# craftsangjae/instance-segmentation-road-project

Hardware: AMD Instinct MI355X
Metric: images/sec at 1024x1024 (MaskLab inference hot path, full forward) (higher is better)
Workload: dtype f32; 1 GPU; resnext50_full_b8_1024; per_gpu_batch=8, global_batch=8, height=1024, width=1024, parallelism=dp1, hipgraph=False, inputs=resident in HBM, weights=random init (cls logits x8 so NMS / mask head run at full load)

## Files before the change

include/masklab_hip.h:

```cpp
#ifndef MASKLAB_HIP_H
#define MASKLAB_HIP_H

#include <stdint.h>

#ifdef __cplusplus
extern "C" {
#endif

#define ML_OK 0
#define ML_E_BADARG (-1)
#define ML_E_LAUNCH (-2)
#define ML_E_NOGPU  (-3)

enum { ML_ACT_NONE = 0, ML_ACT_RELU = 1, ML_ACT_RELU6 = 2, ML_ACT_SIGMOID = 3 };
enum { ML_MATH_F32 = 0, ML_MATH_F16 = 1, ML_MATH_F16S = 2, ML_MATH_F32X3 = 3 };

#define ML_ABI_VERSION 7
int ml_version(void);
const char *ml_last_error(void);
int ml_device_check(void);

typedef struct ml_conv2d_desc {
    const float *in;
    const float *wgt;
// ... 93 lines not shown
                              int32_t B, int32_t H, int32_t W, int32_t C, int32_t in_cstride, int32_t in_coff,
                              int32_t Ho, int32_t Wo, int32_t add_cstride, int32_t add_coff,
                              int32_t out_cstride, int32_t out_coff, void *stream);
int ml_dwconv3x3_f16(const void *in, const float *wgt, const float *bias, void *out,
                     int32_t B, int32_t H, int32_t W, int32_t C, int32_t in_cstride, int32_t in_coff,
                     int32_t out_cstride, int32_t out_coff, int32_t Ho, int32_t Wo,
                     int32_t stride, int32_t dil, int32_t pad_t, int32_t pad_l, int32_t act, void *stream);
int ml_global_mean_f16(const void *in, void *out, int32_t B, int32_t HW, int32_t C, void *stream);

int ml_stem7x7s2_pool_f16(const float *image, const void *wgt_h, const float *bias, void *out, int32_t B, int32_t H,
                          int32_t W, int32_t Hp, int32_t Wp, void *stream);
int ml_stem7x7s2_pool_f32(const float *image, const float *wgt, const float *bias, float *out, int32_t B, int32_t H,
                          int32_t W, int32_t Hp, int32_t Wp, void *stream);
int ml_stem7x7s2_pool_x3(const float *image, const void *wgt_x3, const float *bias, float *out, int32_t B, int32_t H,
                         int32_t W, int32_t Hp, int32_t Wp, void *stream);

typedef struct ml_deconv_out_problem {
    const float *x, *wd, *bd, *wo_table, *bo;
    float *out;
    int64_t M;
    int32_t hw, w, rois_per_image, reserved0;
    int64_t out_image_stride, out_base;
    const int32_t *live;
} ml_deconv_out_problem;
int ml_deconv2x2_out1x1_f32(const ml_deconv_out_problem *probs, int32_t nprob, int32_t K, int32_t c_mid, int32_t ncls,
                            int32_t cp, int32_t act_mid, int32_t act_out, void *stream);
int ml_deconv2x2_out1x1_f16(const ml_deconv_out_problem *probs, int32_t nprob, int32_t K, int32_t c_mid, int32_t ncls,
                            int32_t cp, int32_t act_mid, int32_t act_out, void *stream);
int ml_deconv2x2_out1x1_tape_f32(const ml_deconv_out_problem *probs, float *const *tapes, int32_t nprob, int32_t K,
                                 int32_t c_mid, int32_t ncls, int32_t cp, int32_t act_mid, int32_t act_out, void *stream);
// ... 407 lines not shown
```

instance-segmentation-road-project_amd/csrc/common.h:

```cpp
#pragma once
#include <hip/hip_runtime.h>
#include <stdint.h>
#include <stdio.h>
#include "masklab_hip.h"

typedef float f32x2 __attribute__((ext_vector_type(2)));
typedef float f32x4 __attribute__((ext_vector_type(4)));
typedef float f32x16 __attribute__((ext_vector_type(16)));

typedef _Float16 f16x2 __attribute__((ext_vector_type(2)));
typedef _Float16 f16x4 __attribute__((ext_vector_type(4)));
typedef _Float16 f16x8 __attribute__((ext_vector_type(8)));

typedef unsigned u32x2 __attribute__((ext_vector_type(2)));
typedef unsigned u32x4 __attribute__((ext_vector_type(4)));
typedef int i32x4 __attribute__((ext_vector_type(4)));

void ml_set_error(const char *fmt, ...);

#define ML_REQUIRE(cond, ...)                 \
    do {                                      \
        if (!(cond)) {                        \
            ml_set_error(__VA_ARGS__);        \
            return ML_E_BADARG;               \
// ... 31 lines not shown
            : "+v"(lw[i]) : "v"(hw[i]), "s"(neg_scale), "v"(sv[2 * i + 1]));
    }
    const u32x4 H = {hw[0], hw[1], hw[2], hw[3]}, L = {lw[0], lw[1], lw[2], lw[3]};
    hi = __builtin_bit_cast(f16x8, H);
    lo = __builtin_bit_cast(f16x8, L);
}

__device__ __forceinline__ void split_hi_lo_pair(const float xa, const float xb, const float neg_scale, unsigned &hi, unsigned &lo) {
    const f32x2 x = {xa, xb};
    const f32x2 sc = x * 2048.f;
    hi = __builtin_bit_cast(unsigned, __builtin_convertvector(x, f16x2));
    asm("v_fma_mixlo_f16 %0, %1, %2, %3 op_sel_hi:[1,0,0]" : "=v"(lo) : "v"(hi), "s"(neg_scale), "v"(sc[0]));
    asm("v_fma_mixhi_f16 %0, %1, %2, %3 op_sel:[1,0,0] op_sel_hi:[1,0,0]" : "+v"(lo) : "v"(hi), "s"(neg_scale), "v"(sc[1]));
}

static inline bool ml_aligned16(const void *p) { return (((uintptr_t)p) & 15u) == 0; }

#include <atomic>
static inline int ml_ensure_dynamic_lds(const void *fn, int bytes, std::atomic<unsigned long long> &done,
                                        const char *what) {
    int dev = 0;
    hipError_t e = hipGetDevice(&dev);
    if (e != hipSuccess || dev < 0 || dev >= 64) {
        ml_set_error("%s: hipGetDevice failed or device index %d out of range", what, dev);
        return ML_E_LAUNCH;
    }
    const unsigned long long bit = 1ull << dev;
    if (done.load(std::memory_order_acquire) & bit) return ML_OK;
    e = hipFuncSetAttribute(fn, hipFuncAttributeMaxDynamicSharedMemorySize, bytes);
    if (e != hipSuccess) {
// ... 21 lines not shown
```

instance-segmentation-road-project_amd/csrc/pointwise.hip:

```cpp
#include "common.h"

namespace {

constexpr int TPB = 256;

inline unsigned grid_for(long long n) { return (unsigned)((n + TPB - 1) / TPB); }

struct Affine3 { float m[3], d[3], s[3]; };

__global__ void preprocess_kernel(const void *in, int is_u8, float *out, long long npix, int out_c,
                                  int flip, Affine3 a) {
    const long long i = (long long)blockIdx.x * TPB + threadIdx.x;
    if (i >= npix) return;
    float v[3];
    if (is_u8) {
        const unsigned char *p = reinterpret_cast<const unsigned char *>(in) + i * 3;
        v[0] = p[0]; v[1] = p[1]; v[2] = p[2];
    } else {
        const float *p = reinterpret_cast<const float *>(in) + i * 3;
        v[0] = p[0]; v[1] = p[1]; v[2] = p[2];
    }
    if (flip) { const float t = v[0]; v[0] = v[2]; v[2] = t; }
    const float r0 = (v[0] - a.m[0]) / a.d[0] + a.s[0];
    const float r1 = (v[1] - a.m[1]) / a.d[1] + a.s[1];
    const float r2 = (v[2] - a.m[2]) / a.d[2] + a.s[2];
    if (out_c == 4) {
        f32x4 o = {r0, r1, r2, 0.f};
        *reinterpret_cast<f32x4 *>(out + i * 4) = o;
    } else {
        out[i * 3 + 0] = r0; out[i * 3 + 1] = r1; out[i * 3 + 2] = r2;
    }
}

template <class T> constexpr int VEC = 16 / (int)sizeof(T);

template <class T, int N>
__device__ __forceinline__ void load_f(const T *p, float (&v)[N]) {
    typedef T Tv __attribute__((ext_vector_type(VEC<T>)));
#pragma unroll
    for (int k = 0; k < N / VEC<T>; ++k) {
// ... 378 lines not shown
```

instance-segmentation-road-project_amd/csrc/stem.hip:

```cpp
#include <type_traits>
#include "common.h"

namespace {

constexpr int PTH = 4, PTW = 16;
constexpr int NT = 256;
constexpr int CR = 2 * PTH + 1, CC = 2 * PTW + 1;
constexpr int IR = 2 * (CR - 1) + 7;
constexpr int ICP = 2 * (CC - 1) + 8;
constexpr int NCONV = CR * CC;
constexpr int NSETS = (NCONV + 31) / 32;
constexpr int NIN = (IR * ICP + NT - 1) / NT;
static_assert(NSETS == 10, "the wave -> set map below assumes 10 sets");


struct StemF32 {
    typedef float Wgt;
    typedef float Conv;
    static constexpr bool PAIRED = true;
    static constexpr int CPS = 68;
    static constexpr int IN_BYTES = IR * ICP * 3 * 4;
    float wv[7][4][3];
    __device__ __forceinline__ StemF32(const float *wgt, int nt, int p32, int q) {
#pragma unroll
// ... 124 lines not shown
#pragma unroll
        for (int u = 0; u < NS; ++u) {
            const _Float16 *src = reinterpret_cast<const _Float16 *>(lds) + (ip[u] + 2 * q) * 4;
#pragma unroll
            for (int ky = 0; ky < 7; ++ky) {
                f16x8 xv[2];
#pragma unroll
                for (int s2 = 0; s2 < 2; ++s2) xv[s2] = *reinterpret_cast<const f16x8 *>(src + (ky * ICP + 4 * s2) * 4);
#pragma unroll
                for (int s2 = 0; s2 < 2; ++s2) acc[u] = __builtin_amdgcn_mfma_f32_32x32x16_f16(wv[ky * 2 + s2], xv[s2], acc[u], 0, 0, 0);
            }
        }
    }
};

template <class Math>
constexpr int STEM_LDS = Math::IN_BYTES + NSETS * 32 * Math::CPS * (int)sizeof(typename Math::Conv);

template <class Math>
__device__ __forceinline__ void stem_pool_body(const float *img, const typename Math::Wgt *wgt, const float *bias,
                                               typename Math::Conv *out, int H, int W, int Hc, int Wc, int Hp, int Wp,
                                               int tiles_x, int seg) {
    typedef typename Math::Conv CT;
    typedef CT CTx4 __attribute__((ext_vector_type(4)));
    constexpr int V = 16 / sizeof(CT), NG = 64 / V;
    typedef CT CTxV __attribute__((ext_vector_type(V)));
    constexpr int CPS = Math::CPS;
    extern __shared__ __align__(16) char lds[];
    CT *tconv = reinterpret_cast<CT *>(lds + Math::IN_BYTES);

    const int tid = threadIdx.x, lane = tid & 63, wave = tid >> 6;
    const int p32 = lane & 31, q = lane >> 5;
    const int ty = blockIdx.x, b = blockIdx.y;
    const int py0 = ty * PTH;
    const int cy0 = 2 * py0 - 1;
    const int iy0 = 2 * cy0 - 3;
    const int nt = wave >> 1, s0 = wave & 1;

    const Math m(wgt, nt, p32, q);
    float bv[16];
#pragma unroll
    for (int e = 0; e < 16; ++e) bv[e] = bias ? bias[nt * 32 + (e & 3) + 8 * (e >> 2) + 4 * q] : 0.f;

    int in_c[NIN];
    long long in_off[NIN];
#pragma unroll
    for (int j = 0; j < NIN; ++j) {
        const int i = tid + NT * j;
        const int in_r = i / ICP;
        in_c[j] = i - in_r * ICP;
        const int iy = iy0 + in_r;
        const bool row_ok = i < IR * ICP && (unsigned)iy < (unsigned)H;
        in_off[j] = row_ok ? ((long long)(b * H + iy) * W) * 4 : -1;
    }
    f32x4 stage[NIN];
    auto fetch = [&](int tx) __attribute__((always_inline)) {
        const int ix0 = 2 * (2 * tx * PTW - 1) - 3;
#pragma unroll
        for (int j = 0; j < NIN; ++j) {
            const int ix = ix0 + in_c[j];
            f32x4 v = {0.f, 0.f, 0.f, 0.f};
            if (in_off[j] >= 0 && (unsigned)ix < (unsigned)W) v = *reinterpret_cast<const f32x4 *>(img + in_off[j] + (long long)ix * 4);
            stage[j] = v;
        }
    };
    auto conv_sets = [&](auto nc, int sa, int cx0) __attribute__((always_inline)) {
        constexpr int NS = decltype(nc)::value;
        int ip[NS];
        f32x16 acc[NS];
#pragma unroll
        for (int u = 0; u < NS; ++u) {
            const int cp = min((sa + 2 * u) * 32 + p32, NCONV - 1);
            const int cyl = cp / CC, cxl = cp - cyl * CC;
            ip[u] = (2 * cyl) * ICP + 2 * cxl;
#pragma unroll
            for (int e = 0; e < 16; ++e) acc[u][e] = bv[e];
        }
        m.template products<NS>(lds, ip, q, acc);
// ... 5 lines not shown
            const int cy = cy0 + cyl, cx = cx0 + cxl;
            const bool inside = (unsigned)cy < (unsigned)Hc && (unsigned)cx < (unsigned)Wc;
            CT *dst = tconv + (s * 32 + p32) * CPS + nt * 32 + 4 * q;
#pragma unroll
            for (int e4 = 0; e4 < 4; ++e4) {
                CTx4 v;
#pragma unroll
                for (int e = 0; e < 4; ++e) v[e] = inside ? (CT)fmaxf(acc[u][4 * e4 + e], 0.f) : (CT)0.f;
                *reinterpret_cast<CTx4 *>(dst + 8 * e4) = v;
            }
        }
    };

    const int tx_begin = blockIdx.z * seg, tx_end = min(tiles_x, tx_begin + seg);
    fetch(tx_begin);
    m.deposit(lds, stage, tid);
    __syncthreads();
    for (int tx = tx_begin; tx < tx_end; ++tx) {
        const int px0 = tx * PTW;
        const int cx0 = 2 * px0 - 1;
        if (tx + 1 < tx_end) fetch(tx + 1);

        if constexpr (Math::PAIRED) {
            conv_sets(std::integral_constant<int, 2>{}, s0, cx0);
            conv_sets(std::integral_constant<int, 2>{}, s0 + 4, cx0);
            conv_sets(std::integral_constant<int, 1>{}, s0 + 8, cx0);
        } else {
            for (int s = s0; s < NSETS; s += 2) conv_sets(std::integral_constant<int, 1>{}, s, cx0);
        }
        __syncthreads();

        for (int i = tid; i < PTH * PTW * NG; i += NT) {
            const int cg = i & (NG - 1), pp = i / NG;
            const int ppy = pp / PTW, ppx = pp - ppy * PTW;
            const int oy = py0 + ppy, ox = px0 + ppx;
            if (oy >= Hp || ox >= Wp) continue;
            CTxV mx = *reinterpret_cast<const CTxV *>(tconv + ((2 * ppy) * CC + 2 * ppx) * CPS + cg * V);
#pragma unroll
            for (int dy = 0; dy < 3; ++dy)
#pragma unroll
                for (int dx = 0; dx < 3; ++dx) {
                    if (dy == 0 && dx == 0) continue;
                    const CTxV v = *reinterpret_cast<const CTxV *>(tconv + ((2 * ppy + dy) * CC + 2 * ppx + dx) * CPS + cg * V);
#pragma unroll
                    for (int k = 0; k < V; ++k) mx[k] = v[k] > mx[k] ? v[k] : mx[k];
                }
            *reinterpret_cast<CTxV *>(out + ((long long)(b * Hp + oy) * Wp + ox) * 64 + cg * V) = mx;
        }
        if (tx + 1 < tx_end) m.deposit(lds, stage, tid);
        __syncthreads();
    }
}

__global__ void __launch_bounds__(NT, 1)
stem_pool_f32_kernel(const float *__restrict__ img, const float *__restrict__ wgt, const float *__restrict__ bias,
                     float *__restrict__ out, int H, int W, int Hc, int Wc, int Hp, int Wp, int tiles_x, int seg) {
    stem_pool_body<StemF32>(img, wgt, bias, out, H, W, Hc, Wc, Hp, Wp, tiles_x, seg);
}

__global__ void __launch_bounds__(NT, 1)
stem_pool_x3_kernel(const float *__restrict__ img, const _Float16 *__restrict__ wgt, const float *__restrict__ bias,
                    float *__restrict__ out, int H, int W, int Hc, int Wc, int Hp, int Wp, int tiles_x, int seg) {
    stem_pool_body<StemX3>(img, wgt, bias, out, H, W, Hc, Wc, Hp, Wp, tiles_x, seg);
}

__global__ void __launch_bounds__(NT)
stem_pool_h_kernel(const float *__restrict__ img, const _Float16 *__restrict__ wgt, const float *__restrict__ bias,
                   _Float16 *__restrict__ out, int H, int W, int Hc, int Wc, int Hp, int Wp, int tiles_x, int seg) {
    stem_pool_body<StemH>(img, wgt, bias, out, H, W, Hc, Wc, Hp, Wp, tiles_x, seg);
}

template <class Math>
int stem_pool_launch(void (*kernel)(const float *, const typename Math::Wgt *, const float *, typename Math::Conv *, int, int,
                                    int, int, int, int, int, int),
                     const char *name, const float *image, const void *wgt, const float *bias, void *out, int B, int H, int W,
                     int Hp, int Wp, void *stream) {
    constexpr bool wgt_scalar = std::is_same<typename Math::Wgt, float>::value;
    ML_REQUIRE(image && wgt && out, "%s: null pointer", name);
    ML_REQUIRE(B > 0 && B < 65536 && H > 0 && W > 0, "%s: bad dims", name);
    ML_REQUIRE(ml_aligned16(image) && (wgt_scalar || ml_aligned16(wgt)) && ml_aligned16(out), "%s: %s must be 16-byte aligned",
               name, wgt_scalar ? "image and output" : "pointers");
    const int Hc = (H + 6 - 7) / 2 + 1, Wc = (W + 6 - 7) / 2 + 1;
    ML_REQUIRE(Hp == (Hc + 2 - 3) / 2 + 1 && Wp == (Wc + 2 - 3) / 2 + 1,
               "%s: output must be [B, %d, %d, 64] (ZeroPadding2D(1) + MaxPooling2D(3, 2))", name, (Hc + 2 - 3) / 2 + 1,
               (Wc + 2 - 3) / 2 + 1);
    ML_REQUIRE((long long)B * H * W < (1ll << 31), "%s: too many pixels", name);
    static std::atomic<unsigned long long> lds_ok{0};
    if (int rc = ml_ensure_dynamic_lds(reinterpret_cast<const void *>(kernel), STEM_LDS<Math>, lds_ok, name)) return rc;
    const int tiles_y = (Hp + PTH - 1) / PTH, tiles_x = (Wp + PTW - 1) / PTW;
    int seg = tiles_x;
    while (seg > 1 && (long long)tiles_y * B * ((tiles_x + seg - 1) / seg) < 2ll * ml_resident_blocks(1)) seg = (seg + 1) / 2;
    hipLaunchKernelGGL(kernel, dim3(tiles_y, B, (tiles_x + seg - 1) / seg), dim3(NT), STEM_LDS<Math>, (hipStream_t)stream, image,
                       reinterpret_cast<const typename Math::Wgt *>(wgt), bias, reinterpret_cast<typename Math::Conv *>(out), H, W,
                       Hc, Wc, Hp, Wp, tiles_x, seg);
    ML_CHECK_LAUNCH(name);
    return ML_OK;
}

}

extern "C" int ml_stem7x7s2_pool_f32(const float *image, const float *wgt, const float *bias, float *out, int32_t B, int32_t H,
                                     int32_t W, int32_t Hp, int32_t Wp, void *stream) {
    return stem_pool_launch<StemF32>(stem_pool_f32_kernel, "stem7x7s2_pool_f32", image, wgt, bias, out, B, H, W, Hp, Wp, stream);
}

extern "C" int ml_stem7x7s2_pool_x3(const float *image, const void *wgt_x3, const float *bias, float *out, int32_t B, int32_t H,
                                    int32_t W, int32_t Hp, int32_t Wp, void *stream) {
    return stem_pool_launch<StemX3>(stem_pool_x3_kernel, "stem7x7s2_pool_x3", image, wgt_x3, bias, out, B, H, W, Hp, Wp, stream);
}

extern "C" int ml_stem7x7s2_pool_f16(const float *image, const void *wgt_h, const float *bias, void *out, int32_t B, int32_t H,
                                     int32_t W, int32_t Hp, int32_t Wp, void *stream) {
    return stem_pool_launch<StemH>(stem_pool_h_kernel, "stem7x7s2_pool", image, wgt_h, bias, out, B, H, W, Hp, Wp, stream);
}
```

instance-segmentation-road-project_amd/masklab_hip/_lib.py:

```python
import ctypes as C
import os

_HERE = os.path.dirname(os.path.abspath(__file__))
LIB_PATH = os.path.join(_HERE, "libmasklab_hip.so")

ABI_VERSION = 7
ACT_NONE, ACT_RELU, ACT_RELU6, ACT_SIGMOID = 0, 1, 2, 3
ACT_BY_NAME = {None: ACT_NONE, "linear": ACT_NONE, "relu": ACT_RELU, "relu6": ACT_RELU6,
               "sigmoid": ACT_SIGMOID}


class ConvDesc(C.Structure):
    _fields_ = [
        ("in_", C.c_void_p), ("wgt", C.c_void_p), ("bias", C.c_void_p),
        ("residual", C.c_void_p), ("out", C.c_void_p),
        ("B", C.c_int32), ("H", C.c_int32), ("W", C.c_int32),
        ("in_cstride", C.c_int32), ("in_coff", C.c_int32),
        ("span", C.c_int32), ("span_pad", C.c_int32), ("cpp_shift", C.c_int32),
        ("Ho", C.c_int32), ("Wo", C.c_int32),
        ("KH", C.c_int32), ("KW", C.c_int32), ("stride", C.c_int32), ("dil", C.c_int32),
        ("pad_t", C.c_int32), ("pad_l", C.c_int32),
        ("cout", C.c_int32), ("n_pad", C.c_int32),
        ("out_cstride", C.c_int32), ("out_coff", C.c_int32),
        ("res_cstride", C.c_int32), ("res_coff", C.c_int32),
# ... 130 lines not shown
    "ml_dwconv3x3_dgrad_multi_f32": (C.c_int, [C.POINTER(DwGradDesc), _i32, _vp]),
    "ml_relu_grad_f32": (C.c_int, [_vp, _vp, _vp, _i64, _vp]),
    "ml_deconv2x2_out1x1_f32": (C.c_int, [C.POINTER(DeconvOutProblem), _i32, _i32, _i32, _i32, _i32, _i32, _i32, _vp]),
    "ml_deconv2x2_out1x1_tape_f32": (C.c_int, [C.POINTER(DeconvOutProblem), C.POINTER(C.c_void_p)] + [_i32] * 7 + [_vp]),
    "ml_deconv2x2_out1x1_grad_f32": (C.c_int, [C.POINTER(DeconvOutGradProblem), _i32, _i32, _vp, _i64, _vp]),
    "ml_deconv2x2_out1x1_grad_plan": (C.c_int, [C.POINTER(DeconvOutGradProblem), _i32, C.POINTER(C.c_int32), C.POINTER(C.c_int32),
                                                C.POINTER(C.c_int64)]),
    "ml_deconv2x2_grad_relayout_f32": (C.c_int, [_vp, _vp, _vp, _vp, _i32, _i32, _vp]),
    "ml_gconv3x3_f32": (C.c_int, [_vp, _vp, _vp, _vp] + [_i32] * 11 + [_vp]),
    "ml_gconv3x3_f16": (C.c_int, [_vp, _vp, _vp, _vp] + [_i32] * 11 + [_vp]),
    "ml_gconv3x3_launch_plan": (C.c_int, [_i32] * 9 + [C.POINTER(C.c_int32)]),
    "ml_maxpool3x3s2_f16": (C.c_int, [_vp, _vp] + [_i32] * 8 + [_vp]),
    "ml_stem7x7s2_pool_f16": (C.c_int, [_vp, _vp, _vp, _vp] + [_i32] * 5 + [_vp]),
    "ml_stem7x7s2_pool_f32": (C.c_int, [_vp, _vp, _vp, _vp] + [_i32] * 5 + [_vp]),
    "ml_stem7x7s2_pool_x3": (C.c_int, [_vp, _vp, _vp, _vp] + [_i32] * 5 + [_vp]),
    "ml_subsample2_f16": (C.c_int, [_vp, _vp] + [_i32] * 4 + [_vp]),
    "ml_cast_f16_to_f32": (C.c_int, [_vp, _vp, _i64, _vp]),
    "ml_cast_f32_to_f16": (C.c_int, [_vp, _vp, _i64, _vp]),
    "ml_resize_bilinear_ac_f16": (C.c_int, [_vp, _vp, _vp] + [_i32] * 12 + [_vp]),
    "ml_dwconv3x3_f16": (C.c_int, [_vp, _vp, _vp, _vp] + [_i32] * 15 + [_vp]),
    "ml_global_mean_f16": (C.c_int, [_vp, _vp, _i32, _i32, _i32, _vp]),
    "ml_groupnorm_chunk_f16": (C.c_int, [_vp, _vp, _vp, _vp, _i32, _i64, _i32, _i32, _f32, _i32, _i32, _i32, _vp, _vp]),
    "ml_roi_crop_resize_f16": (C.c_int, [_vp, _vp, _i32, _i32, _vp, _vp, _vp, _vp] + [_i32] * 10 + [_f32, _f32, _i32, _i32, _vp, _vp]),
    "ml_deconv2x2_out1x1_f16": (C.c_int, [C.POINTER(DeconvOutProblem), _i32, _i32, _i32, _i32, _i32, _i32, _i32, _vp]),
    "ml_dwconv3x3_f32": (C.c_int, [_vp, _vp, _vp, _vp] + [_i32] * 15 + [_vp]),
    "ml_maxpool3x3s2_f32": (C.c_int, [_vp, _vp] + [_i32] * 8 + [_vp]),
    "ml_preprocess_f32": (C.c_int, [_vp, _i32, _vp, _i64, _i32, _i32, C.POINTER(C.c_float), C.POINTER(C.c_float),
                                    C.POINTER(C.c_float), _vp]),
    "ml_groupnorm_workspace_bytes": (_i64, [_i32, _i32]),
    "ml_groupnorm_multi_f32": (C.c_int, [C.POINTER(GnDesc), _i32, _vp, _i64, _vp]),
# ... 139 lines not shown
```

instance-segmentation-road-project_amd/masklab_hip/backbone/base.py:

```python
from .. import ops
from ..keras_like import Conv2D, DepthwiseConv2D, GroupedConv2D, Layer
from ..layers.misc import Identity
from ..normalization import GroupNormalization
from .body import input_affine
from .mobilenet import MobileNetV1
from .resnet50 import ResNet50
from .resnext import ResNeXt50
from .resnext101 import ResNeXt101
from .senet import SEResNet50, SEResNeXt50
from .seresnet34 import SEResNet34

BACKBONE_LAYERS = {
    "resnet50": {"C1": 'activation', "C2": 'activation_9', "C3": "activation_21", "C4": "activation_39",
                 "C5": "activation_48"},
    "resnext50": {"C1": 'conv1_relu', "C2": 'conv2_block3_out', "C3": "conv3_block4_out",
                  "C4": "conv4_block6_out", "C5": "conv5_block3_out"},
    "resnext101": {"C1": "relu0", "C2": "stage1_unit3_relu", "C3": "stage2_unit4_relu",
                   "C4": "stage3_unit23_relu", "C5": "stage4_unit3_relu"},
    "seresnet34": {"C1": "relu0", "C2": "stage2_unit1_relu1", "C3": "stage3_unit1_relu1", "C4": "stage4_unit1_relu1",
                   "C5": "relu1"},
    "seresnet50": {"C1": "activation", "C2": "activation_15", "C3": "activation_35", "C4": "activation_65",
                   "C5": "activation_80"},
    "seresnext50": {"C1": "activation", "C2": "activation_16", "C3": "activation_36", "C4": "activation_66",
                    "C5": "activation_80"},
# ... 16 lines not shown

    def __init__(self, rgb=True, mean_shift=False, normalize=0, out_channels=4, **kwargs):
        self.rgb = rgb
        self.mean_shift = mean_shift
        self.normalize = normalize
        self.out_channels = out_channels
        super().__init__(**kwargs)
        self.mean = [123.68, 116.779, 103.939] if rgb else [103.939, 116.779, 123.68]
        self.std = [0.225, 0.224, 0.229] if rgb else [0.229, 0.224, 0.225]
        self.extra_affine = None

    def build(self, input_shape):
        self.built = True
        return tuple(input_shape[:3]) + (self.out_channels,)

    def call(self, inputs, **kwargs):
        mean = self.mean if self.mean_shift else [0.0, 0.0, 0.0]
        if self.normalize == 1:
            div, shift = 255.0, 0.0
        elif self.normalize == 2:
            div, shift = 127.5, (0.0 if self.mean_shift else -1.0)
        elif self.normalize == 3:
            div, shift = [255.0 * s for s in self.std], 0.0
        else:
            div, shift = 1.0, 0.0
        if self.extra_affine is not None:
            if self.normalize != 0 or self.mean_shift:
                raise NotImplementedError("an input BatchNorm is only combined with the raw (normalize=0) mode")
            mean, div, shift = self.extra_affine
        return ops.preprocess(inputs, flip=not self.rgb, mean=mean, divisor=div, shift=shift,
                              out_channels=self.out_channels)

    def get_config(self):
        config = super().get_config()
        config.update({"rgb": self.rgb, "mean_shift": self.mean_shift, "normalize": self.normalize})
        return config


class BackboneModel(Layer):

    def __init__(self, backbone_type, backbone_outputs, num_features, **kwargs):
        super().__init__(name=backbone_type, **kwargs)
        bt = backbone_type.lower()
        if bt not in BACKBONES:
            raise NotImplementedError(
                f"backbone_type must be one of {list(BACKBONES)} on the MI355X path (got '{backbone_type}')")
# ... 36 lines not shown
        return [self.body, self.p6_conv, self.p6_norm, self.p7_conv]

    def weight_specs(self):
        out = {}
        for ch in self.children():
            out.update(ch.weight_specs())
        return out

    def load_weights(self, weights, device):
        super().load_weights(weights, device)
        eps = getattr(self.body, "INPUT_BN_EPS", None)
        if eps is not None:
            self.preprocess.extra_affine = input_affine(weights, eps)

    def call(self, images, **kwargs):
        x = self.preprocess(images)
        taps = self.body(x, wanted=self.taps)
        feats = [self.identities[k](taps[k]) for k in self.taps]
        fork = kwargs.get("fork_stream")
        aux = fork("_extra_level_stream") if fork is not None else None
        self.pending_stream = aux
        import contextlib
        import torch
        with (torch.cuda.stream(aux) if aux is not None else contextlib.nullcontext()):
            p6 = self.p6_conv(feats[-1])
            g6 = self.p6_norm(p6)
            p7 = self.p7_conv(g6)
        if 'P6' in self.backbone_outputs:
            feats.append(p6)
        if 'P7' in self.backbone_outputs:
            feats.append(p7)
        return feats
# ... 24 lines not shown
```

instance-segmentation-road-project_amd/masklab_hip/backbone/body.py:

```python
import numpy as np

from .. import ops
from ..keras_like import Layer, WeightSpec

STAGE_TAPS = ("C2", "C3", "C4", "C5")


def bn_data_specs():
    return {
        "bn_data/beta": WeightSpec((3,), "normal", stddev=0.1),
        "bn_data/moving_mean": WeightSpec((3,), "uniform", low=100.0, high=130.0),
        "bn_data/moving_variance": WeightSpec((3,), "uniform", low=3000.0, high=5000.0),
    }


def input_affine(weights, eps):
    mean = np.asarray(weights["bn_data/moving_mean"], np.float64)
    div = np.sqrt(np.asarray(weights["bn_data/moving_variance"], np.float64) + eps)
    return mean.astype(np.float32), div.astype(np.float32), np.asarray(weights["bn_data/beta"], np.float32)


class BatchNorm(Layer):

    def __init__(self, channels, eps, gamma_range=(0.5, 1.5), **kwargs):
# ... 62 lines not shown
        taps = {}
        for tap, stage in zip(STAGE_TAPS, self.stages):
            for u in stage:
                s = u.build(s)
            taps[tap] = s
        return taps

    def children(self):
        return [self.stem] + [l for u in self.units() for l in u.layers()] + list(self.trailing)

    def weight_specs(self):
        out = bn_data_specs() if self.INPUT_BN_EPS is not None else {}
        out.update(super().weight_specs())
        return out

    def call(self, x, wanted=("C3", "C4", "C5"), **kwargs):
        import torch
        half = ops.half_storage()
        taps = {}
        if "C1" not in wanted and self.stem.dev is not None and ops.has_fused_stem():
            x = ops.stem_pool(x, self.stem.dev)
        else:
            x = self.stem(x, out_dtype=torch.float16 if half else None)
            taps["C1"] = x
            x = ops.maxpool3x3s2(x, pad=1)
        last = max(int(t[1]) for t in wanted)
        if last >= 2:
            self.run_stages(x, taps, last)
        return taps

    def run_stages(self, x, taps, last):
        for tap, stage in zip(STAGE_TAPS, self.stages):
            if int(tap[1]) > last:
                break
            for u in stage:
# ... 3 lines not shown
```

instance-segmentation-road-project_amd/masklab_hip/ops.py:

```python
import ctypes as C
import dataclasses
import threading

import numpy as np
import torch

from . import _lib
from .packing import (NO_PIX_SPAN, PackedConv, dgrad_padding, pack_dense_transposed, pack_winograd, resolve_padding,
                      transposed_geometry, unpack_dense)

import weakref

_ws_cache = {}
_ws_retired = []
_graph_owners = weakref.WeakSet()


def graph_owner_registered(model):
    _graph_owners.add(model)


def graph_owner_released(model):
    _graph_owners.discard(model)
    if not len(_graph_owners):
# ... 721 lines not shown
    elif out.dtype != x.dtype:
        raise ValueError("dwconv3x3: out must have the input's dtype")
    fn = lib.ml_dwconv3x3_f16 if half else lib.ml_dwconv3x3_f32
    with _Prof("dwconv3x3_h" if half else "dwconv3x3", 18.0 * B * Ho * Wo * Cc,
               x.element_size() * (x.numel() + B * Ho * Wo * Cc) + 4 * 9 * Cc):
        _lib.check(fn(_ptr(x), _ptr(wgt), _ptr(bias), _ptr(out), B, H, W, Cc, Cc, 0,
                      out.shape[3], out_coff, Ho, Wo, stride, dilation, pt, pl, act, _stream()), "ml_dwconv3x3")
    return out


def has_fused_stem():
    return CONV_MATH in ("f32", "f32x3", "f16s")


def stem_pool(x4, dc: "DeviceConv"):
    lib = _lib.load()
    _require_dev(x4, "x4")
    p = dc.p
    B, H, W, c4 = x4.shape
    if x4.dtype != torch.float32 or c4 != 4 or p.cpp_shift == 30 or p.KH != 7 or p.span_pad != 32 or p.cout != 64 or p.n_pad != 64:
        raise ValueError("stem_pool: needs the fp32 NHWC4 image and the 7x7 / 64-filter row-span stem packing")
    if not has_fused_stem():
        raise ValueError(f"stem_pool: no fused stem in conv math {CONV_MATH!r}")
    if CONV_MATH == "f16s":
        label, fn, w, dtype = "stem7x7s2_pool_h", lib.ml_stem7x7s2_pool_f16, dc.wgt_stem_h, torch.float16
    elif CONV_MATH == "f32x3":
        label, fn, w, dtype = "stem7x7s2_pool_x3", lib.ml_stem7x7s2_pool_x3, dc.wgt_x3, torch.float32
    else:
        label, fn, w, dtype = "stem7x7s2_pool", lib.ml_stem7x7s2_pool_f32, dc.wgt, torch.float32
    Hc, Wc = (H + 6 - 7) // 2 + 1, (W + 6 - 7) // 2 + 1
    Hp, Wp = (Hc + 2 - 3) // 2 + 1, (Wc + 2 - 3) // 2 + 1
    out = torch.empty((B, Hp, Wp, 64), dtype=dtype, device=x4.device)
    es = out.element_size()
    with _Prof(label, 2.0 * B * Hc * Wc * 64 * 147, 16 * B * H * W + es * out.numel() + es * 64 * 224,
               f"B={B} HxW={H}x{W} -> {Hp}x{Wp}x64"):
        _lib.check(fn(_ptr(x4), _ptr(w), _ptr(dc.bias), _ptr(out), B, H, W, Hp, Wp, _stream()), "ml_stem7x7s2_pool")
    return out


def maxpool3x3s2(x, pad=1):
    lib = _lib.load()
    _require_dev(x, "x")
    B, H, W, Cc = x.shape
    Ho = (H + 2 * pad - 3) // 2 + 1
    Wo = (W + 2 * pad - 3) // 2 + 1
    half = x.dtype == torch.float16
    out = torch.empty((B, Ho, Wo, Cc), dtype=x.dtype, device=x.device)
    fn = lib.ml_maxpool3x3s2_f16 if half else lib.ml_maxpool3x3s2_f32
    with _Prof("maxpool3x3s2_h" if half else "maxpool3x3s2", 0, x.element_size() * (x.numel() + out.numel())):
        _lib.check(fn(_ptr(x), _ptr(out), B, H, W, Cc, Ho, Wo, pad, pad, _stream()), "ml_maxpool3x3s2")
    return out
# ... 30 lines not shown
    out = torch.empty(x.shape, dtype=torch.float16, device=x.device)
    with _Prof("cast_f2h", 0, 6 * x.numel()):
        _lib.check(lib.ml_cast_f32_to_f16(_ptr(x), _ptr(out), x.numel(), _stream()), "ml_cast_f32_to_f16")
    return out


def preprocess(images, flip, mean, divisor, shift, out_channels=4):
    lib = _lib.load()
    _require_dev(images, "images")
    if images.dtype not in (torch.uint8, torch.float32):
        raise TypeError("images must be uint8 or float32")
    B, H, W, ch = images.shape
    if ch != 3:
        raise ValueError("images must have 3 channels (RGB, 0..255)")
    out = torch.empty((B, H, W, out_channels), dtype=torch.float32, device=images.device)
    f3 = C.c_float * 3
    div3 = [float(divisor)] * 3 if np.isscalar(divisor) else [float(v) for v in divisor]
    sh3 = [float(shift)] * 3 if np.isscalar(shift) else [float(v) for v in shift]
    with _Prof("preprocess", 0, images.numel() * images.element_size() + 4 * out.numel()):
        _lib.check(lib.ml_preprocess_f32(_ptr(images), int(images.dtype == torch.uint8), _ptr(out), B * H * W,
                                         out_channels, int(flip), f3(*[float(m) for m in mean]), f3(*div3), f3(*sh3),
                                         _stream()), "ml_preprocess_f32")
    return out


def _gn_output(x, out, out_coff, dtype):
    _require_dev(x, "x")
    if out is None:
        out = torch.empty_like(x)
    _require_dev(out, "out")
    if out.shape[-1] == x.shape[-1]:
        if out.numel() != x.numel() or out_coff != 0:
            raise ValueError("groupnorm: dense output must match the input size")
    elif tuple(out.shape[:-1]) != tuple(x.shape[:-1]):
        raise ValueError("groupnorm: concat buffer spatial shape mismatch")
    if out.dtype != x.dtype or x.dtype != dtype or x.dtype not in (torch.float32, torch.float16):
        raise ValueError("groupnorm: every x / out of one launch must share a dtype (float32 or float16)")
# ... 2253 lines not shown
```

instance-segmentation-road-project_amd/masklab_hip/retinamasklab.py:

```python
import numpy as np
import torch

from . import backbone
from . import keras_like as K
from .config import ModelConfiguration
from .layers import (ASPPNetwork, AssignBoxes, AssignMasks, AssignSeg, BoxRegressionSubNet, ClassificationSubNet, CropAndPadMask,
                     DetectionProposal,
                     DownSampleInput, DrawBoxes, DrawInstance, DrawSegmentation, EncodeImageContent, SummaryOutput,
                     FeaturePyramid, MaskDistribute, MaskSubNet, PriorLayer, PyramidRoiAlign, ResizeLike,
                     RestoreBoxes, SegmentationSubNet, SemanticSmoothing, TrimInstances, UpSampleOutput)
from .prior import PriorBoxes

VERBOSE = False


def _say(*lines):
    if VERBOSE:
        print("\n".join(lines))


def construct_masklabdataset(configuration: ModelConfiguration, device="cuda"):
    from .utils import MaskLabDataset
    d_config = configuration.dataset
    trainset, validset = (MaskLabDataset(cases, min_area=d_config.min_area, data_dir=d_config.data_dir,
# ... 365 lines not shown
    def enable_graphs(self, enabled=True):
        self._use_graphs = bool(enabled)
        if not enabled:
            self._drop_graphs()
        return self

    @property
    def outputs_graph_owned(self):
        return bool(self._use_graphs)

    def _stage1_graphed(self, images, whole=False):
        from . import ops
        dp = self.detection_proposal
        key = (tuple(images.shape), images.dtype, ops.CONV_MATH, bool(whole)) + (
            () if dp is None else (float(dp.min_confidence), float(dp.nms_iou_threshold), float(dp.post_iou_threshold),
                                   int(dp.nms_max_output_size)))
        entry = self._graphs.get(key)
        if entry is None:
            if ops.PROFILE is not None:
                raise RuntimeError("graph capture cannot run under the per-launch profiling hook")
            if whole:
                self._stage2_capacity(self._stage1(images))
            else:
                self._join_side(self._stage1(images))
            torch.cuda.synchronize(self.device)
            static_in = images.clone()
            graph = torch.cuda.CUDAGraph()
            self._capturing_whole = bool(whole)
            try:
                with torch.cuda.graph(graph):
                    st = self._stage1(static_in)
# ... 511 lines not shown
```

Baseline: 436.7 images/sec.

## Fuse uint8 preprocessing into the stem conv+pool kernel

```diff
diff --git a/include/masklab_hip.h b/include/masklab_hip.h
--- a/include/masklab_hip.h
+++ b/include/masklab_hip.h
@@ -131,6 +131,15 @@
                           int32_t W, int32_t Hp, int32_t Wp, void *stream);
 int ml_stem7x7s2_pool_x3(const float *image, const void *wgt_x3, const float *bias, float *out, int32_t B, int32_t H,
                          int32_t W, int32_t Hp, int32_t Wp, void *stream);
+int ml_stem_pool_u8_f32(const uint8_t *image, const float *wgt, const float *bias, float *out, int32_t B, int32_t H,
+                        int32_t W, int32_t Hp, int32_t Wp, int32_t flip, const float *mean, const float *div,
+                        const float *shift, void *stream);
+int ml_stem_pool_u8_x3(const uint8_t *image, const void *wgt_x3, const float *bias, float *out, int32_t B, int32_t H,
+                       int32_t W, int32_t Hp, int32_t Wp, int32_t flip, const float *mean, const float *div,
+                       const float *shift, void *stream);
+int ml_stem_pool_u8_f16(const uint8_t *image, const void *wgt_h, const float *bias, void *out, int32_t B, int32_t H,
+                        int32_t W, int32_t Hp, int32_t Wp, int32_t flip, const float *mean, const float *div,
+                        const float *shift, void *stream);
 
 typedef struct ml_deconv_out_problem {
     const float *x, *wd, *bd, *wo_table, *bo;
diff --git a/instance-segmentation-road-project_amd/csrc/common.h b/instance-segmentation-road-project_amd/csrc/common.h
--- a/instance-segmentation-road-project_amd/csrc/common.h
+++ b/instance-segmentation-road-project_amd/csrc/common.h
@@ -69,6 +69,11 @@
     asm("v_fma_mixhi_f16 %0, %1, %2, %3 op_sel:[1,0,0] op_sel_hi:[1,0,0]" : "+v"(lo) : "v"(hi), "s"(neg_scale), "v"(sc[1]));
 }
 
+struct Affine3 { float m[3], d[3], s[3]; };
+__device__ __forceinline__ float ml_affine3(float v, const Affine3 &a, int k) {
+    return (v - a.m[k]) / a.d[k] + a.s[k];
+}
+
 static inline bool ml_aligned16(const void *p) { return (((uintptr_t)p) & 15u) == 0; }
 
 #include <atomic>
diff --git a/instance-segmentation-road-project_amd/csrc/pointwise.hip b/instance-segmentation-road-project_amd/csrc/pointwise.hip
--- a/instance-segmentation-road-project_amd/csrc/pointwise.hip
+++ b/instance-segmentation-road-project_amd/csrc/pointwise.hip
@@ -5,8 +5,6 @@
 constexpr int TPB = 256;
 
 inline unsigned grid_for(long long n) { return (unsigned)((n + TPB - 1) / TPB); }
-
-struct Affine3 { float m[3], d[3], s[3]; };
 
 __global__ void preprocess_kernel(const void *in, int is_u8, float *out, long long npix, int out_c,
                                   int flip, Affine3 a) {
@@ -21,9 +19,7 @@
         v[0] = p[0]; v[1] = p[1]; v[2] = p[2];
     }
     if (flip) { const float t = v[0]; v[0] = v[2]; v[2] = t; }
-    const float r0 = (v[0] - a.m[0]) / a.d[0] + a.s[0];
-    const float r1 = (v[1] - a.m[1]) / a.d[1] + a.s[1];
-    const float r2 = (v[2] - a.m[2]) / a.d[2] + a.s[2];
+    const float r0 = ml_affine3(v[0], a, 0), r1 = ml_affine3(v[1], a, 1), r2 = ml_affine3(v[2], a, 2);
     if (out_c == 4) {
         f32x4 o = {r0, r1, r2, 0.f};
         *reinterpret_cast<f32x4 *>(out + i * 4) = o;
diff --git a/instance-segmentation-road-project_amd/csrc/stem.hip b/instance-segmentation-road-project_amd/csrc/stem.hip
--- a/instance-segmentation-road-project_amd/csrc/stem.hip
+++ b/instance-segmentation-road-project_amd/csrc/stem.hip
@@ -1,5 +1,10 @@
 #include <type_traits>
 #include "common.h"
+#include "gfx_mem.h"
+
+#ifndef STEM_EXP
+#define STEM_EXP 0
+#endif
 
 namespace {
 
@@ -162,13 +167,13 @@
     }
 };
 
-template <class Math>
-constexpr int STEM_LDS = Math::IN_BYTES + NSETS * 32 * Math::CPS * (int)sizeof(typename Math::Conv);
-
-template <class Math>
-__device__ __forceinline__ void stem_pool_body(const float *img, const typename Math::Wgt *wgt, const float *bias,
+template <class Math, bool U8>
+constexpr int STEM_LDS = Math::IN_BYTES + NSETS * 32 * Math::CPS * (int)sizeof(typename Math::Conv) + (U8 ? 3 * 256 * 4 : 0);
+
+template <class Math, bool U8>
+__device__ __forceinline__ void stem_pool_body(const void *img_, const typename Math::Wgt *wgt, const float *bias,
                                                typename Math::Conv *out, int H, int W, int Hc, int Wc, int Hp, int Wp,
-                                               int tiles_x, int seg) {
+                                               int tiles_x, int seg, const Affine3 &aff, int flip) {
     typedef typename Math::Conv CT;
     typedef CT CTx4 __attribute__((ext_vector_type(4)));
     constexpr int V = 16 / sizeof(CT), NG = 64 / V;
@@ -176,6 +181,9 @@
     constexpr int CPS = Math::CPS;
     extern __shared__ __align__(16) char lds[];
     CT *tconv = reinterpret_cast<CT *>(lds + Math::IN_BYTES);
+    float *tab = reinterpret_cast<float *>(lds + STEM_LDS<Math, false>);
+    constexpr int PXB = U8 ? 3 : 16;
+    typedef std::conditional_t<U8, unsigned, f32x4> Stage;
 
     const int tid = threadIdx.x, lane = tid & 63, wave = tid >> 6;
     const int p32 = lane & 31, q = lane >> 5;
@@ -199,17 +207,43 @@
         in_c[j] = i - in_r * ICP;
         const int iy = iy0 + in_r;
         const bool row_ok = i < IR * ICP && (unsigned)iy < (unsigned)H;
-        in_off[j] = row_ok ? ((long long)(b * H + iy) * W) * 4 : -1;
-    }
-    f32x4 stage[NIN];
+        in_off[j] = row_ok ? ((long long)(b * H + iy) * W) * PXB : -1;
+    }
+    Stage stage[NIN];
+    unsigned inside = 0;
     auto fetch = [&](int tx) __attribute__((always_inline)) {
         const int ix0 = 2 * (2 * tx * PTW - 1) - 3;
+        if constexpr (U8) inside = 0;
 #pragma unroll
         for (int j = 0; j < NIN; ++j) {
             const int ix = ix0 + in_c[j];
-            f32x4 v = {0.f, 0.f, 0.f, 0.f};
-            if (in_off[j] >= 0 && (unsigned)ix < (unsigned)W) v = *reinterpret_cast<const f32x4 *>(img + in_off[j] + (long long)ix * 4);
-            stage[j] = v;
+            const bool ok = in_off[j] >= 0 && (unsigned)ix < (unsigned)W;
+            if constexpr (U8) {
+                const long long off = ok ? in_off[j] + (long long)ix * 3 : 0;
+                const bool first = off == 0;
+                __builtin_memcpy(&stage[j], reinterpret_cast<const char *>(img_) + (first ? 0 : off - 1), 4);
+                inside |= (ok ? 1u : 0u) << j | (first ? 0x100u : 0u) << j;
+            } else {
+                f32x4 v = {0.f, 0.f, 0.f, 0.f};
+                if (ok) v = *reinterpret_cast<const f32x4 *>(reinterpret_cast<const char *>(img_) + in_off[j] + (long long)ix * PXB);
+                stage[j] = v;
+            }
+        }
+    };
+    auto deposit = [&]() __attribute__((always_inline)) {
+        if constexpr (U8) {
+            f32x4 px[NIN];
+#pragma unroll
+            for (int j = 0; j < NIN; ++j) {
+                const unsigned v = stage[j] >> (inside >> (8 + j) & 1 ? 0 : 8);
+                const unsigned c0 = v & 255, c1 = v >> 8 & 255, c2 = v >> 16 & 255;
+                const float r0 = tab[flip ? c2 : c0], r1 = tab[256 + c1], r2 = tab[512 + (flip ? c0 : c2)];
+                const bool in = inside >> j & 1;
+                px[j] = f32x4{in ? r0 : 0.f, in ? r1 : 0.f, in ? r2 : 0.f, 0.f};
+            }
+            m.deposit(lds, px, tid);
+        } else {
+            m.deposit(lds, stage, tid);
         }
     };
     auto conv_sets = [&](auto nc, int sa, int cx0) __attribute__((always_inline)) {
@@ -245,7 +279,11 @@
 
     const int tx_begin = blockIdx.z * seg, tx_end = min(tiles_x, tx_begin + seg);
     fetch(tx_begin);
-    m.deposit(lds, stage, tid);
+    if constexpr (U8) {
+        for (int i = tid; i < 3 * 256; i += NT) tab[i] = ml_affine3((float)(i & 255), aff, i >> 8);
+        __syncthreads();
+    }
+    deposit();
     __syncthreads();
     for (int tx = tx_begin; tx < tx_end; ++tx) {
         const int px0 = tx * PTW;
@@ -266,6 +304,11 @@
             const int ppy = pp / PTW, ppx = pp - ppy * PTW;
             const int oy = py0 + ppy, ox = px0 + ppx;
             if (oy >= Hp || ox >= Wp) continue;
+#if STEM_EXP == 1
+            CTxV mx;
+#pragma unroll
+            for (int k = 0; k < V; ++k) mx[k] = (CT)0.f;
+#else
             CTxV mx = *reinterpret_cast<const CTxV *>(tconv + ((2 * ppy) * CC + 2 * ppx) * CPS + cg * V);
 #pragma unroll
             for (int dy = 0; dy < 3; ++dy)
@@ -276,9 +319,21 @@
 #pragma unroll
                     for (int k = 0; k < V; ++k) mx[k] = v[k] > mx[k] ? v[k] : mx[k];
                 }
-            *reinterpret_cast<CTxV *>(out + ((long long)(b * Hp + oy) * Wp + ox) * 64 + cg * V) = mx;
-        }
-        if (tx + 1 < tx_end) m.deposit(lds, stage, tid);
+#endif
+            const long long o = ((long long)(b * Hp + oy) * Wp + ox) * 64 + cg * V;
+#if STEM_EXP == 3 && defined(__HIP_DEVICE_COMPILE__)
+            __builtin_amdgcn_raw_buffer_store_b128(__builtin_bit_cast(u32x4, mx), rsrc_bytes(out, 0), (int)(o * sizeof(CT)), 0, 0);
+#else
+            *reinterpret_cast<CTxV *>(out + o) = mx;
+#endif
+        }
+#if STEM_EXP == 2
+        if (tx + 1 < tx_end)
+#pragma unroll
+            for (int j = 0; j < NIN; ++j) asm volatile("" ::"v"(stage[j]));
+#else
+        if (tx + 1 < tx_end) deposit();
+#endif
         __syncthreads();
     }
 }
@@ -286,44 +341,69 @@
 __global__ void __launch_bounds__(NT, 1)
 stem_pool_f32_kernel(const float *__restrict__ img, const float *__restrict__ wgt, const float *__restrict__ bias,
                      float *__restrict__ out, int H, int W, int Hc, int Wc, int Hp, int Wp, int tiles_x, int seg) {
-    stem_pool_body<StemF32>(img, wgt, bias, out, H, W, Hc, Wc, Hp, Wp, tiles_x, seg);
+    stem_pool_body<StemF32, false>(img, wgt, bias, out, H, W, Hc, Wc, Hp, Wp, tiles_x, seg, Affine3{}, 0);
 }
 
 __global__ void __launch_bounds__(NT, 1)
 stem_pool_x3_kernel(const float *__restrict__ img, const _Float16 *__restrict__ wgt, const float *__restrict__ bias,
                     float *__restrict__ out, int H, int W, int Hc, int Wc, int Hp, int Wp, int tiles_x, int seg) {
-    stem_pool_body<StemX3>(img, wgt, bias, out, H, W, Hc, Wc, Hp, Wp, tiles_x, seg);
+    stem_pool_body<StemX3, false>(img, wgt, bias, out, H, W, Hc, Wc, Hp, Wp, tiles_x, seg, Affine3{}, 0);
 }
 
 __global__ void __launch_bounds__(NT)
 stem_pool_h_kernel(const float *__restrict__ img, const _Float16 *__restrict__ wgt, const float *__restrict__ bias,
                    _Float16 *__restrict__ out, int H, int W, int Hc, int Wc, int Hp, int Wp, int tiles_x, int seg) {
-    stem_pool_body<StemH>(img, wgt, bias, out, H, W, Hc, Wc, Hp, Wp, tiles_x, seg);
-}
-
-template <class Math>
-int stem_pool_launch(void (*kernel)(const float *, const typename Math::Wgt *, const float *, typename Math::Conv *, int, int,
-                                    int, int, int, int, int, int),
-                     const char *name, const float *image, const void *wgt, const float *bias, void *out, int B, int H, int W,
-                     int Hp, int Wp, void *stream) {
+    stem_pool_body<StemH, false>(img, wgt, bias, out, H, W, Hc, Wc, Hp, Wp, tiles_x, seg, Affine3{}, 0);
+}
+
+__global__ void __launch_bounds__(NT, 1)
+stem_pool_u8_f32_kernel(const unsigned char *__restrict__ img, const float *__restrict__ wgt, const float *__restrict__ bias,
+                        float *__restrict__ out, int H, int W, int Hc, int Wc, int Hp, int Wp, int tiles_x, int seg, Affine3 a,
+                        int flip) {
+    stem_pool_body<StemF32, true>(img, wgt, bias, out, H, W, Hc, Wc, Hp, Wp, tiles_x, seg, a, flip);
+}
+
+__global__ void __launch_bounds__(NT, 1)
+stem_pool_u8_x3_kernel(const unsigned char *__restrict__ img, const _Float16 *__restrict__ wgt, const float *__restrict__ bias,
+                       float *__restrict__ out, int H, int W, int Hc, int Wc, int Hp, int Wp, int tiles_x, int seg, Affine3 a,
+                       int flip) {
+    stem_pool_body<StemX3, true>(img, wgt, bias, out, H, W, Hc, Wc, Hp, Wp, tiles_x, seg, a, flip);
+}
+
+__global__ void __launch_bounds__(NT)
+stem_pool_u8_h_kernel(const unsigned char *__restrict__ img, const _Float16 *__restrict__ wgt, const float *__restrict__ bias,
+                      _Float16 *__restrict__ out, int H, int W, int Hc, int Wc, int Hp, int Wp, int tiles_x, int seg, Affine3 a,
+                      int flip) {
+    stem_pool_body<StemH, true>(img, wgt, bias, out, H, W, Hc, Wc, Hp, Wp, tiles_x, seg, a, flip);
+}
+
+template <class Math, class Img, class... Extra>
+int stem_pool_launch(void (*kernel)(const Img *, const typename Math::Wgt *, const float *, typename Math::Conv *, int, int,
+                                    int, int, int, int, int, int, Extra...),
+                     const char *name, const Img *image, const void *wgt, const float *bias, void *out, int B, int H, int W,
+                     int Hp, int Wp, void *stream, Extra... extra) {
     constexpr bool wgt_scalar = std::is_same<typename Math::Wgt, float>::value;
+    constexpr bool U8 = std::is_same<Img, unsigned char>::value;
     ML_REQUIRE(image && wgt && out, "%s: null pointer", name);
     ML_REQUIRE(B > 0 && B < 65536 && H > 0 && W > 0, "%s: bad dims", name);
-    ML_REQUIRE(ml_aligned16(image) && (wgt_scalar || ml_aligned16(wgt)) && ml_aligned16(out), "%s: %s must be 16-byte aligned",
-               name, wgt_scalar ? "image and output" : "pointers");
+    ML_REQUIRE((U8 || ml_aligned16(image)) && (wgt_scalar || ml_aligned16(wgt)) && ml_aligned16(out),
+               "%s: %s must be 16-byte aligned", name,
+               U8 ? (wgt_scalar ? "output" : "weights and output") : wgt_scalar ? "image and output" : "pointers");
     const int Hc = (H + 6 - 7) / 2 + 1, Wc = (W + 6 - 7) / 2 + 1;
     ML_REQUIRE(Hp == (Hc + 2 - 3) / 2 + 1 && Wp == (Wc + 2 - 3) / 2 + 1,
                "%s: output must be [B, %d, %d, 64] (ZeroPadding2D(1) + MaxPooling2D(3, 2))", name, (Hc + 2 - 3) / 2 + 1,
                (Wc + 2 - 3) / 2 + 1);
     ML_REQUIRE((long long)B * H * W < (1ll << 31), "%s: too many pixels", name);
+    ML_REQUIRE(!U8 || (long long)B * H * W >= 2, "%s: a uint8 image of two pixels or more (4-byte loads)", name);
     static std::atomic<unsigned long long> lds_ok{0};
-    if (int rc = ml_ensure_dynamic_lds(reinterpret_cast<const void *>(kernel), STEM_LDS<Math>, lds_ok, name)) return rc;
+    constexpr int lds_bytes = STEM_LDS<Math, U8>;
+    if (int rc = ml_ensure_dynamic_lds(reinterpret_cast<const void *>(kernel), lds_bytes, lds_ok, name)) return rc;
     const int tiles_y = (Hp + PTH - 1) / PTH, tiles_x = (Wp + PTW - 1) / PTW;
     int seg = tiles_x;
     while (seg > 1 && (long long)tiles_y * B * ((tiles_x + seg - 1) / seg) < 2ll * ml_resident_blocks(1)) seg = (seg + 1) / 2;
-    hipLaunchKernelGGL(kernel, dim3(tiles_y, B, (tiles_x + seg - 1) / seg), dim3(NT), STEM_LDS<Math>, (hipStream_t)stream, image,
-                       reinterpret_cast<const typename Math::Wgt *>(wgt), bias, reinterpret_cast<typename Math::Conv *>(out), H, W,
-                       Hc, Wc, Hp, Wp, tiles_x, seg);
+    hipLaunchKernelGGL(kernel, dim3(tiles_y, B, (tiles_x + seg - 1) / seg), dim3(NT), lds_bytes, (hipStream_t)stream,
+                       image, reinterpret_cast<const typename Math::Wgt *>(wgt), bias,
+                       reinterpret_cast<typename Math::Conv *>(out), H, W, Hc, Wc, Hp, Wp, tiles_x, seg, extra...);
     ML_CHECK_LAUNCH(name);
     return ML_OK;
 }
@@ -344,3 +424,37 @@
                                      int32_t W, int32_t Hp, int32_t Wp, void *stream) {
     return stem_pool_launch<StemH>(stem_pool_h_kernel, "stem7x7s2_pool", image, wgt_h, bias, out, B, H, W, Hp, Wp, stream);
 }
+
+namespace {
+template <class Math, class K>
+int stem_pool_u8(K kernel, const char *name, const uint8_t *image, const void *wgt, const float *bias, void *out, int B, int H,
+                 int W, int Hp, int Wp, int flip, const float *mean, const float *div, const float *shift, void *stream) {
+    ML_REQUIRE(mean && div && shift, "%s: null pointer", name);
+    ML_REQUIRE(div[0] != 0.f && div[1] != 0.f && div[2] != 0.f, "%s: zero divisor", name);
+    Affine3 a;
+    for (int k = 0; k < 3; ++k) { a.m[k] = mean[k]; a.d[k] = div[k]; a.s[k] = shift[k]; }
+    return stem_pool_launch<Math, unsigned char, Affine3, int>(kernel, name, image, wgt, bias, out, B, H, W, Hp, Wp, stream, a,
+                                                               flip ? 1 : 0);
+}
+}
+
+extern "C" int ml_stem_pool_u8_f32(const uint8_t *image, const float *wgt, const float *bias, float *out, int32_t B, int32_t H,
+                                   int32_t W, int32_t Hp, int32_t Wp, int32_t flip, const float *mean, const float *div,
+                                   const float *shift, void *stream) {
+    return stem_pool_u8<StemF32>(stem_pool_u8_f32_kernel, "stem_pool_u8_f32", image, wgt, bias, out, B, H, W, Hp, Wp, flip, mean,
+                                 div, shift, stream);
+}
+
+extern "C" int ml_stem_pool_u8_x3(const uint8_t *image, const void *wgt_x3, const float *bias, float *out, int32_t B, int32_t H,
+                                  int32_t W, int32_t Hp, int32_t Wp, int32_t flip, const float *mean, const float *div,
+                                  const float *shift, void *stream) {
+    return stem_pool_u8<StemX3>(stem_pool_u8_x3_kernel, "stem_pool_u8_x3", image, wgt_x3, bias, out, B, H, W, Hp, Wp, flip, mean,
+                                div, shift, stream);
+}
+
+extern "C" int ml_stem_pool_u8_f16(const uint8_t *image, const void *wgt_h, const float *bias, void *out, int32_t B, int32_t H,
+                                   int32_t W, int32_t Hp, int32_t Wp, int32_t flip, const float *mean, const float *div,
+                                   const float *shift, void *stream) {
+    return stem_pool_u8<StemH>(stem_pool_u8_h_kernel, "stem_pool_u8_f16", image, wgt_h, bias, out, B, H, W, Hp, Wp, flip, mean,
+                               div, shift, stream);
+}
diff --git a/instance-segmentation-road-project_amd/masklab_hip/_lib.py b/instance-segmentation-road-project_amd/masklab_hip/_lib.py
--- a/instance-segmentation-road-project_amd/masklab_hip/_lib.py
+++ b/instance-segmentation-road-project_amd/masklab_hip/_lib.py
@@ -168,6 +168,9 @@
     "ml_stem7x7s2_pool_f16": (C.c_int, [_vp, _vp, _vp, _vp] + [_i32] * 5 + [_vp]),
     "ml_stem7x7s2_pool_f32": (C.c_int, [_vp, _vp, _vp, _vp] + [_i32] * 5 + [_vp]),
     "ml_stem7x7s2_pool_x3": (C.c_int, [_vp, _vp, _vp, _vp] + [_i32] * 5 + [_vp]),
+    "ml_stem_pool_u8_f16": (C.c_int, [_vp, _vp, _vp, _vp] + [_i32] * 6 + [C.POINTER(C.c_float)] * 3 + [_vp]),
+    "ml_stem_pool_u8_f32": (C.c_int, [_vp, _vp, _vp, _vp] + [_i32] * 6 + [C.POINTER(C.c_float)] * 3 + [_vp]),
+    "ml_stem_pool_u8_x3": (C.c_int, [_vp, _vp, _vp, _vp] + [_i32] * 6 + [C.POINTER(C.c_float)] * 3 + [_vp]),
     "ml_subsample2_f16": (C.c_int, [_vp, _vp] + [_i32] * 4 + [_vp]),
     "ml_cast_f16_to_f32": (C.c_int, [_vp, _vp, _i64, _vp]),
     "ml_cast_f32_to_f16": (C.c_int, [_vp, _vp, _i64, _vp]),
diff --git a/instance-segmentation-road-project_amd/masklab_hip/backbone/base.py b/instance-segmentation-road-project_amd/masklab_hip/backbone/base.py
--- a/instance-segmentation-road-project_amd/masklab_hip/backbone/base.py
+++ b/instance-segmentation-road-project_amd/masklab_hip/backbone/base.py
@@ -54,7 +54,7 @@
         self.built = True
         return tuple(input_shape[:3]) + (self.out_channels,)
 
-    def call(self, inputs, **kwargs):
+    def affine(self):
         mean = self.mean if self.mean_shift else [0.0, 0.0, 0.0]
         if self.normalize == 1:
             div, shift = 255.0, 0.0
@@ -68,8 +68,11 @@
             if self.normalize != 0 or self.mean_shift:
                 raise NotImplementedError("an input BatchNorm is only combined with the raw (normalize=0) mode")
             mean, div, shift = self.extra_affine
-        return ops.preprocess(inputs, flip=not self.rgb, mean=mean, divisor=div, shift=shift,
-                              out_channels=self.out_channels)
+        return (not self.rgb), mean, div, shift
+
+    def call(self, inputs, **kwargs):
+        flip, mean, div, shift = self.affine()
+        return ops.preprocess(inputs, flip=flip, mean=mean, divisor=div, shift=shift, out_channels=self.out_channels)
 
     def get_config(self):
         config = super().get_config()
@@ -136,8 +139,11 @@
             self.preprocess.extra_affine = input_affine(weights, eps)
 
     def call(self, images, **kwargs):
-        x = self.preprocess(images)
-        taps = self.body(x, wanted=self.taps)
+        fuses_stem = getattr(self.body, "fuses_stem", None)
+        if fuses_stem is not None and fuses_stem(self.taps) and ops.stem_reads_bytes(images):
+            taps = self.body(images, wanted=self.taps, raw_affine=self.preprocess.affine())
+        else:
+            taps = self.body(self.preprocess(images), wanted=self.taps)
         feats = [self.identities[k](taps[k]) for k in self.taps]
         fork = kwargs.get("fork_stream")
         aux = fork("_extra_level_stream") if fork is not None else None
diff --git a/instance-segmentation-road-project_amd/masklab_hip/backbone/body.py b/instance-segmentation-road-project_amd/masklab_hip/backbone/body.py
--- a/instance-segmentation-road-project_amd/masklab_hip/backbone/body.py
+++ b/instance-segmentation-road-project_amd/masklab_hip/backbone/body.py
@@ -100,11 +100,18 @@
         out.update(super().weight_specs())
         return out
 
-    def call(self, x, wanted=("C3", "C4", "C5"), **kwargs):
+    def fuses_stem(self, wanted):
+        return "C1" not in wanted and self.stem.dev is not None and ops.has_fused_stem()
+
+    def call(self, x, wanted=("C3", "C4", "C5"), raw_affine=None, **kwargs):
         import torch
         half = ops.half_storage()
         taps = {}
-        if "C1" not in wanted and self.stem.dev is not None and ops.has_fused_stem():
+        if raw_affine is not None:
+            if not self.fuses_stem(wanted):
+                raise ValueError("a raw uint8 image needs the fused stem (no C1 tap, weights loaded, a conv math that has one)")
+            x = ops.stem_pool_u8(x, self.stem.dev, *raw_affine)
+        elif self.fuses_stem(wanted):
             x = ops.stem_pool(x, self.stem.dev)
         else:
             x = self.stem(x, out_dtype=torch.float16 if half else None)
diff --git a/instance-segmentation-road-project_amd/masklab_hip/ops.py b/instance-segmentation-road-project_amd/masklab_hip/ops.py
--- a/instance-segmentation-road-project_amd/masklab_hip/ops.py
+++ b/instance-segmentation-road-project_amd/masklab_hip/ops.py
@@ -759,27 +759,61 @@
 
 
 def stem_pool(x4, dc: "DeviceConv"):
-    lib = _lib.load()
-    _require_dev(x4, "x4")
+    return _stem_pool(x4, dc, None)
+
+
+STEM_INPUT = "u8"
+
+
+def set_stem_input(mode):
+    global STEM_INPUT
+    if mode not in ("u8", "f32"):
+        raise ValueError(f"stem input must be 'u8' or 'f32', got {mode!r}")
+    STEM_INPUT = mode
+
+
+def stem_reads_bytes(images):
+    return STEM_INPUT == "u8" and images.dtype == torch.uint8 and has_fused_stem() and images.numel() >= 6
+
+
+def affine3(mean, divisor, shift):
+    f3 = C.c_float * 3
+    div3 = [float(divisor)] * 3 if np.isscalar(divisor) else [float(v) for v in divisor]
+    sh3 = [float(shift)] * 3 if np.isscalar(shift) else [float(v) for v in shift]
+    return f3(*[float(m) for m in mean]), f3(*div3), f3(*sh3)
+
+
+def stem_pool_u8(images, dc: "DeviceConv", flip, mean, divisor, shift):
+    return _stem_pool(images, dc, (int(bool(flip)),) + affine3(mean, divisor, shift))
+
+
+def _stem_pool(x, dc, pre):
+    lib = _lib.load()
+    what = "stem_pool" if pre is None else "stem_pool_u8"
+    _require_dev(x, "x4" if pre is None else "images")
     p = dc.p
-    B, H, W, c4 = x4.shape
-    if x4.dtype != torch.float32 or c4 != 4 or p.cpp_shift == 30 or p.KH != 7 or p.span_pad != 32 or p.cout != 64 or p.n_pad != 64:
-        raise ValueError("stem_pool: needs the fp32 NHWC4 image and the 7x7 / 64-filter row-span stem packing")
+    B, H, W, ch = x.shape
+    bad_image = (x.dtype != torch.float32 or ch != 4) if pre is None else (x.dtype != torch.uint8 or ch != 3)
+    if bad_image or p.cpp_shift == 30 or p.KH != 7 or p.span_pad != 32 or p.cout != 64 or p.n_pad != 64:
+        raise ValueError(f"{what}: needs the {'fp32 NHWC4' if pre is None else 'uint8 [B,H,W,3]'} image and the 7x7 / 64-filter "
+                         "row-span stem packing")
     if not has_fused_stem():
-        raise ValueError(f"stem_pool: no fused stem in conv math {CONV_MATH!r}")
+        raise ValueError(f"{what}: no fused stem in conv math {CONV_MATH!r}")
     if CONV_MATH == "f16s":
-        label, fn, w, dtype = "stem7x7s2_pool_h", lib.ml_stem7x7s2_pool_f16, dc.wgt_stem_h, torch.float16
+        label, sfx, w, dtype = "stem7x7s2_pool_h", "f16", dc.wgt_stem_h, torch.float16
     elif CONV_MATH == "f32x3":
-        label, fn, w, dtype = "stem7x7s2_pool_x3", lib.ml_stem7x7s2_pool_x3, dc.wgt_x3, torch.float32
+        label, sfx, w, dtype = "stem7x7s2_pool_x3", "x3", dc.wgt_x3, torch.float32
     else:
-        label, fn, w, dtype = "stem7x7s2_pool", lib.ml_stem7x7s2_pool_f32, dc.wgt, torch.float32
+        label, sfx, w, dtype = "stem7x7s2_pool", "f32", dc.wgt, torch.float32
+    fn = getattr(lib, ("ml_stem7x7s2_pool_" if pre is None else "ml_stem_pool_u8_") + sfx)
     Hc, Wc = (H + 6 - 7) // 2 + 1, (W + 6 - 7) // 2 + 1
     Hp, Wp = (Hc + 2 - 3) // 2 + 1, (Wc + 2 - 3) // 2 + 1
-    out = torch.empty((B, Hp, Wp, 64), dtype=dtype, device=x4.device)
+    out = torch.empty((B, Hp, Wp, 64), dtype=dtype, device=x.device)
     es = out.element_size()
-    with _Prof(label, 2.0 * B * Hc * Wc * 64 * 147, 16 * B * H * W + es * out.numel() + es * 64 * 224,
-               f"B={B} HxW={H}x{W} -> {Hp}x{Wp}x64"):
-        _lib.check(fn(_ptr(x4), _ptr(w), _ptr(dc.bias), _ptr(out), B, H, W, Hp, Wp, _stream()), "ml_stem7x7s2_pool")
+    with _Prof(label, 2.0 * B * Hc * Wc * 64 * 147, (16 if pre is None else 3) * B * H * W + es * out.numel() + es * 64 * 224,
+               f"B={B} HxW={H}x{W} -> {Hp}x{Wp}x64" + ("" if pre is None else " u8")):
+        _lib.check(fn(_ptr(x), _ptr(w), _ptr(dc.bias), _ptr(out), B, H, W, Hp, Wp, *(pre or ()), _stream()),
+                   "ml_stem7x7s2_pool" if pre is None else "ml_stem_pool_u8")
     return out
 
 
@@ -840,13 +874,10 @@
     if ch != 3:
         raise ValueError("images must have 3 channels (RGB, 0..255)")
     out = torch.empty((B, H, W, out_channels), dtype=torch.float32, device=images.device)
-    f3 = C.c_float * 3
-    div3 = [float(divisor)] * 3 if np.isscalar(divisor) else [float(v) for v in divisor]
-    sh3 = [float(shift)] * 3 if np.isscalar(shift) else [float(v) for v in shift]
     with _Prof("preprocess", 0, images.numel() * images.element_size() + 4 * out.numel()):
         _lib.check(lib.ml_preprocess_f32(_ptr(images), int(images.dtype == torch.uint8), _ptr(out), B * H * W,
-                                         out_channels, int(flip), f3(*[float(m) for m in mean]), f3(*div3), f3(*sh3),
-                                         _stream()), "ml_preprocess_f32")
+                                         out_channels, int(flip), *affine3(mean, divisor, shift), _stream()),
+                   "ml_preprocess_f32")
     return out
 
 
diff --git a/instance-segmentation-road-project_amd/masklab_hip/retinamasklab.py b/instance-segmentation-road-project_amd/masklab_hip/retinamasklab.py
--- a/instance-segmentation-road-project_amd/masklab_hip/retinamasklab.py
+++ b/instance-segmentation-road-project_amd/masklab_hip/retinamasklab.py
@@ -403,7 +403,7 @@
         dp = self.detection_proposal
         key = (tuple(images.shape), images.dtype, ops.CONV_MATH, bool(whole)) + (
             () if dp is None else (float(dp.min_confidence), float(dp.nms_iou_threshold), float(dp.post_iou_threshold),
-                                   int(dp.nms_max_output_size)))
+                                   int(dp.nms_max_output_size))) + (ops.STEM_INPUT,)
         entry = self._graphs.get(key)
         if entry is None:
             if ops.PROFILE is not None:
```

Result: no change. 433.9 images/sec (-0.6%).
